# hongfz16/Garment4D

Hardware: AMD Instinct MI355X
Metric: point-cloud frames/s (FPS+ball_query+SA-MLP+LBS), B=8 N=8192 (higher is better)
Workload: dtype f32

## Files before the change

### garment4d_amd/csrc/three_nn_prune.hip

```cpp
#include <cstdlib>

#include "g4d_common.h"
#include "three_nn_body.h"
#include "ball_grid_build.h"

namespace g4d {

namespace {
constexpr int kPrM = 1024;
constexpr int kPrBlk = 16;
constexpr int kPrNB = kPrM / kPrBlk;

__device__ __forceinline__ unsigned pr_part1by2(unsigned v) {
    v &= 0x3ffu;
    v = (v | (v << 16)) & 0x030000ffu;
    v = (v | (v << 8)) & 0x0300f00fu;
    v = (v | (v << 4)) & 0x030c30c3u;
    v = (v | (v << 2)) & 0x09249249u;
    return v;
}

__device__ __forceinline__ float pr_wave_min(float v) {
#pragma unroll
    for (int o = 32; o > 0; o >>= 1) v = fminf(v, __shfl_xor(v, o));
    return v;
}
__device__ __forceinline__ float pr_wave_max(float v) {
#pragma unroll
    for (int o = 32; o > 0; o >>= 1) v = fmaxf(v, __shfl_xor(v, o));
    return v;
}
}

constexpr size_t kPrBoxOff = (size_t)kPrM * 16, kPrCodeOff = kPrBoxOff + (size_t)kPrNB * 32, kPrGridOff = kPrCodeOff + (size_t)kPrNB * 4;
constexpr size_t kPrCloudBytes = kPrGridOff + 16;
constexpr int kPrepT = 512;

__global__ void __launch_bounds__(kPrepT) nn_prune_prep_kernel(int m, const float *__restrict__ known_all, unsigned char *__restrict__ ws) {
    __shared__ unsigned long long keys[kPrM];
    __shared__ float sx[kPrM], sy[kPrM], sz[kPrM];
    __shared__ float red[6][kPrepT / 64];
    const int t = threadIdx.x, lane = t & 63, wave = t >> 6, b = blockIdx.x;
    const float *known = known_all + (size_t)b * m * 3;
    const float INF = __builtin_inff();
    float lx = INF, ly = INF, lz = INF, hx = -INF, hy = -INF, hz = -INF;
    for (int k = t; k < kPrM; k += kPrepT) {
        const bool ok = k < m;
        const float x = ok ? known[k * 3 + 0] : INF, y = ok ? known[k * 3 + 1] : INF, z = ok ? known[k * 3 + 2] : INF;
        sx[k] = x; sy[k] = y; sz[k] = z;
        if (ok && x - x == 0.f && y - y == 0.f && z - z == 0.f) {
            lx = fminf(lx, x); ly = fminf(ly, y); lz = fminf(lz, z);
            hx = fmaxf(hx, x); hy = fmaxf(hy, y); hz = fmaxf(hz, z);
        }
    }
    lx = pr_wave_min(lx); ly = pr_wave_min(ly); lz = pr_wave_min(lz);
    hx = pr_wave_max(hx); hy = pr_wave_max(hy); hz = pr_wave_max(hz);
    if (lane == 0) { red[0][wave] = lx; red[1][wave] = ly; red[2][wave] = lz; red[3][wave] = hx; red[4][wave] = hy; red[5][wave] = hz; }
    __syncthreads();
#pragma unroll
    for (int w = 0; w < kPrepT / 64; ++w) {
        lx = fminf(lx, red[0][w]); ly = fminf(ly, red[1][w]); lz = fminf(lz, red[2][w]);
        hx = fmaxf(hx, red[3][w]); hy = fmaxf(hy, red[4][w]); hz = fmaxf(hz, red[5][w]);
    }
    const float ext = fmaxf(fmaxf(hx - lx, hy - ly), fmaxf(hz - lz, 1e-30f));
    const float scale = ext < INF ? 1023.0f / ext : 0.f;
    for (int k = t; k < kPrM; k += kPrepT) {
        unsigned long long key = ~0ull;
        if (k < m) {
            const float x = sx[k], y = sy[k], z = sz[k];
            const unsigned cx = (unsigned)fminf(fmaxf((x - lx) * scale, 0.f), 1023.f);
            const unsigned cy = (unsigned)fminf(fmaxf((y - ly) * scale, 0.f), 1023.f);
            const unsigned cz = (unsigned)fminf(fmaxf((z - lz) * scale, 0.f), 1023.f);
            const unsigned code = pr_part1by2(cx) | (pr_part1by2(cy) << 1) | (pr_part1by2(cz) << 2);
            key = ((unsigned long long)code << 32) | (unsigned)k;
        }
        keys[k] = key;
    }
    __syncthreads();
    for (int k = 2; k <= kPrM; k <<= 1) {
        for (int j = k >> 1; j > 0; j >>= 1) {
            for (int i = t; i < kPrM / 2; i += kPrepT) {
                const int a = ((i & ~(j - 1)) << 1) | (i & (j - 1));
                const int c = a | j;
                const unsigned long long ka = keys[a], kc = keys[c];
                const bool asc = (a & k) == 0;
                if ((ka > kc) == asc) { keys[a] = kc; keys[c] = ka; }
            }
            __syncthreads();
        }
    }
    float4 *rec = reinterpret_cast<float4 *>(ws + (size_t)b * kPrCloudBytes);
    float *box = reinterpret_cast<float *>(ws + (size_t)b * kPrCloudBytes + kPrBoxOff);
    unsigned *bcode = reinterpret_cast<unsigned *>(ws + (size_t)b * kPrCloudBytes + kPrCodeOff);
    if (t == 0) { float *g = reinterpret_cast<float *>(ws + (size_t)b * kPrCloudBytes + kPrGridOff); g[0] = lx; g[1] = ly; g[2] = lz; g[3] = scale; }
    for (int p = t; p < kPrM; p += kPrepT) {
        const unsigned long long key = keys[p];
        const bool ok = key != ~0ull;
        const int k = ok ? (int)(unsigned)key : 0;
        rec[p] = make_float4(ok ? sx[k] : INF, ok ? sy[k] : INF, ok ? sz[k] : INF, __int_as_float(ok ? k : 0x7fffffff));
    }
    if (t < kPrNB) {
        float bl[3] = {INF, INF, INF}, bh[3] = {-INF, -INF, -INF};
        for (int q = 0; q < kPrBlk; ++q) {
            const unsigned long long key = keys[t * kPrBlk + q];
            if (key == ~0ull) continue;
            const int k = (int)(unsigned)key;
            bl[0] = fminf(bl[0], sx[k]); bl[1] = fminf(bl[1], sy[k]); bl[2] = fminf(bl[2], sz[k]);
            bh[0] = fmaxf(bh[0], sx[k]); bh[1] = fmaxf(bh[1], sy[k]); bh[2] = fmaxf(bh[2], sz[k]);
        }
        bcode[t] = (unsigned)(keys[t * kPrBlk] >> 32);
        float *o = box + t * 8;
        o[0] = bl[0]; o[1] = bl[1]; o[2] = bl[2]; o[3] = 0.f; o[4] = bh[0]; o[5] = bh[1]; o[6] = bh[2]; o[7] = 0.f;
    }
}

__device__ __forceinline__ float pr_gap(float lo, float hi, float qlo, float qhi) { return fmaxf(fmaxf(lo - qhi, qlo - hi), 0.f); }

constexpr int kPrT = 1024;
template <int FM>
__global__ void __launch_bounds__(kPrT) three_nn_prune_kernel(int n, int m, const float *__restrict__ unknown_all, const unsigned char *__restrict__ ws,
                                                            float *__restrict__ dist2_all, int *__restrict__ idx_all,
                                                            const unsigned char *__restrict__ qrec, size_t qstride, int sorted_out) {
    constexpr int LB = kPrBlk + 4;
    __shared__ __attribute__((aligned(16))) float skx[kPrNB * LB], sky[kPrNB * LB], skz[kPrNB * LB];
    __shared__ __attribute__((aligned(16))) int ski[kPrNB * LB];
    __shared__ __attribute__((aligned(16))) float sbox[kPrNB * 8];
    __shared__ unsigned scode[kPrNB];
    __shared__ float sgrid[4];
    const int b = blockIdx.y, t = threadIdx.x, lane = t & 63;
    static_assert(kPrM == kPrT && kPrNB * 8 <= kPrT, "one record per thread");
    const unsigned char *cw = ws + (size_t)b * kPrCloudBytes;
    const float4 r = reinterpret_cast<const float4 *>(cw)[t];
    const float boxv = reinterpret_cast<const float *>(cw + kPrBoxOff)[min(t, kPrNB * 8 - 1)];
    const unsigned codev = reinterpret_cast<const unsigned *>(cw + kPrCodeOff)[min(t, kPrNB - 1)];
    const float gridv = reinterpret_cast<const float *>(cw + kPrGridOff)[min(t, 3)];
    const int p = (int)blockIdx.x * kPrT + t;
    float ux, uy, uz;
    int orig = p;
    if (qrec) {
        const float4 q = reinterpret_cast<const float4 *>(qrec + (size_t)b * qstride)[min(p, n - 1)];
        ux = q.x; uy = q.y; uz = q.z; orig = sorted_out ? p : __float_as_int(q.w);
    } else {
        const float *u = unknown_all + ((size_t)b * n + min(p, n - 1)) * 3;
        ux = u[0]; uy = u[1]; uz = u[2];
    }
    {
        const int jj = (t >> 4) * LB + (t & 15);
        skx[jj] = r.x; sky[jj] = r.y; skz[jj] = r.z; ski[jj] = __float_as_int(r.w);
        if (t < kPrNB * 8) sbox[t] = boxv;
        if (t < kPrNB) scode[t] = codev;
        if (t < 4) sgrid[t] = gridv;
    }
    __syncthreads();
    const float INF = __builtin_inff();
    float b1 = INF, b2 = INF, b3 = INF;
    int i1 = 0, i2 = 0, i3 = 0;
    const int nblk = (m + kPrBlk - 1) / kPrBlk;
    int hb;
    {
        const float gx = sgrid[0], gy = sgrid[1], gz = sgrid[2], gs = sgrid[3];
        const unsigned cx = (unsigned)fminf(fmaxf((ux - gx) * gs, 0.f), 1023.f), cy = (unsigned)fminf(fmaxf((uy - gy) * gs, 0.f), 1023.f),
                       cz = (unsigned)fminf(fmaxf((uz - gz) * gs, 0.f), 1023.f);
        const unsigned cq = pr_part1by2(cx) | (pr_part1by2(cy) << 1) | (pr_part1by2(cz) << 2);
        int pos = 0;
#pragma unroll
        for (int step = kPrNB / 2; step > 0; step >>= 1)
            if (pos + step < nblk && scode[pos + step] <= cq) pos += step;
        hb = pos;
#pragma unroll 4
        for (int s4 = 0; s4 < kPrBlk; ++s4) {
            const int j = hb * LB + s4;
            const float d = dist2<FM>(ux - skx[j], uy - sky[j], uz - skz[j]);
            if (d < INF) nn_insert_lex(d, ski[j], b1, b2, b3, i1, i2, i3);
        }
    }
    const float qlx = pr_wave_min(ux), qly = pr_wave_min(uy), qlz = pr_wave_min(uz);
    const float qhx = pr_wave_max(ux), qhy = pr_wave_max(uy), qhz = pr_wave_max(uz);
    const float *mybox = sbox + min(lane, kPrNB - 1) * 8;
    const float wbound = dist2<FM>(pr_gap(mybox[0], mybox[4], qlx, qhx), pr_gap(mybox[1], mybox[5], qly, qhy), pr_gap(mybox[2], mybox[6], qlz, qhz));
    const bool nanq = !(ux == ux && uy == uy && uz == uz);
    const float maxb3 = pr_wave_max(nanq ? -INF : b3);
    unsigned long long rest = __builtin_amdgcn_ballot_w64(lane < nblk && !(wbound > maxb3));
    for (; rest != 0ull; rest &= rest - 1) {
        const int blk = __builtin_ctzll(rest);
        const float *bx = sbox + blk * 8;
        const float dq = dist2<FM>(pr_gap(bx[0], bx[4], ux, ux), pr_gap(bx[1], bx[5], uy, uy), pr_gap(bx[2], bx[6], uz, uz));
        const bool want = !nanq && blk != hb && !(dq > b3);
        if (__builtin_amdgcn_ballot_w64(want) == 0ull) continue;
#pragma unroll
        for (int s4 = 0; s4 < kPrBlk; s4 += 4) {
            const int j = blk * LB + s4;
            const float4 kx = *reinterpret_cast<const float4 *>(&skx[j]), ky = *reinterpret_cast<const float4 *>(&sky[j]),
                         kz = *reinterpret_cast<const float4 *>(&skz[j]);
            const int4 ki = *reinterpret_cast<const int4 *>(&ski[j]);
            const float d0 = dist2<FM>(ux - kx.x, uy - ky.x, uz - kz.x);
            const float d1 = dist2<FM>(ux - kx.y, uy - ky.y, uz - kz.y);
            const float d2 = dist2<FM>(ux - kx.z, uy - ky.z, uz - kz.z);
            const float d3 = dist2<FM>(ux - kx.w, uy - ky.w, uz - kz.w);
            const bool ok = blk != hb;
            if (__builtin_amdgcn_ballot_w64(ok && fminf(fminf(d0, d1), fminf(d2, d3)) <= b3) == 0ull) continue;
            if (__builtin_amdgcn_ballot_w64(ok && d0 <= b3 && d0 < INF) != 0ull) { if (ok && d0 < INF) nn_insert_lex(d0, ki.x, b1, b2, b3, i1, i2, i3); }
            if (__builtin_amdgcn_ballot_w64(ok && d1 <= b3 && d1 < INF) != 0ull) { if (ok && d1 < INF) nn_insert_lex(d1, ki.y, b1, b2, b3, i1, i2, i3); }
            if (__builtin_amdgcn_ballot_w64(ok && d2 <= b3 && d2 < INF) != 0ull) { if (ok && d2 < INF) nn_insert_lex(d2, ki.z, b1, b2, b3, i1, i2, i3); }
            if (__builtin_amdgcn_ballot_w64(ok && d3 <= b3 && d3 < INF) != 0ull) { if (ok && d3 < INF) nn_insert_lex(d3, ki.w, b1, b2, b3, i1, i2, i3); }
        }
    }
    if (p < n) {
        float *d2o = dist2_all + ((size_t)b * n + orig) * 3;
        int *ix = idx_all + ((size_t)b * n + orig) * 3;
        d2o[0] = b1; d2o[1] = b2; d2o[2] = b3;
        ix[0] = i1; ix[1] = i2; ix[2] = i3;
    }
}

}

using namespace g4d;

extern "C" int g4d_three_nn_pruned_supported(int n, int m) { return n > 0 && m >= 16 && m <= kPrM; }
extern "C" long long g4d_three_nn_pruned_ws_bytes(int b) { return (long long)(b > 0 ? b : 0) * (long long)kPrCloudBytes; }
extern "C" int g4d_three_nn_pruned_f32(int b, int n, int m, const float *unknown, const void *unknown_grid, const float *known, float *dist2, int *idx,
                                       int sorted_out, void *ws, long long ws_bytes, g4d_stream_t stream) {
    G4D_REQUIRE(b >= 0 && b <= 65535 && g4d_three_nn_pruned_supported(n, m), "g4d_three_nn_pruned_f32: needs 16 <= m <= 1024, n > 0, b <= 65535 (use g4d_three_nn_f32)");
    if (b == 0) return G4D_OK;
    G4D_REQUIRE(known && dist2 && idx && ws && (unknown || unknown_grid) && (!sorted_out || unknown_grid), "g4d_three_nn_pruned_f32: null pointer");
    G4D_REQUIRE(ws_bytes >= g4d_three_nn_pruned_ws_bytes(b) && (reinterpret_cast<uintptr_t>(ws) & 15) == 0, "g4d_three_nn_pruned_f32: workspace too small or not 16-byte aligned");
    hipStream_t st = reinterpret_cast<hipStream_t>(stream);
    hipLaunchKernelGGL(nn_prune_prep_kernel, dim3(b), dim3(kPrepT), 0, st, m, known, reinterpret_cast<unsigned char *>(ws));
    if (const int rc = check_launch("g4d_three_nn_pruned_f32(prep)")) return rc;
    size_t off = 0, stride = 0;
    const unsigned char *qrec = nullptr;
    if (unknown_grid) {
        grid_sorted_layout(n, &off, &stride);
        qrec = reinterpret_cast<const unsigned char *>(unknown_grid) + off;
    }
    dim3 grid((n + kPrT - 1) / kPrT, b);
    G4D_WITH_FM(distance_contraction(), hipLaunchKernelGGL((three_nn_prune_kernel<FM>), grid, dim3(kPrT), 0, st, n, m, unknown, reinterpret_cast<const unsigned char *>(ws), dist2, idx,
                                                           qrec, stride, sorted_out))
    return check_launch("g4d_three_nn_pruned_f32");
}
```

Before: 52110.

## Compact per-wave candidate point lists before three-NN refinement in pruned kernel

Replaces the block-by-block refinement loop with a two-round scheme. Each wavefront gathers candidate known points from surviving blocks, filtering them per point against the wave's bounding box and a distance threshold, and writes the survivors into a shared-memory list via ballot/mbcnt compaction. All lanes then scan this dense list. The first round uses the wave-min of the current third-best distance and the second round the wave-max, which aims to reduce wasted distance evaluations and divergence. The cost is extra shared memory (which may lower occupancy), wave-level barriers, and more complex control flow.

```diff
diff --git a/garment4d_amd/csrc/three_nn_prune.hip b/garment4d_amd/csrc/three_nn_prune.hip
--- a/garment4d_amd/csrc/three_nn_prune.hip
+++ b/garment4d_amd/csrc/three_nn_prune.hip
@@ -116,6 +116,13 @@
 
 __device__ __forceinline__ float pr_gap(float lo, float hi, float qlo, float qhi) { return fmaxf(fmaxf(lo - qhi, qlo - hi), 0.f); }
 
+__device__ __forceinline__ void pr_wave_sync() {
+    __builtin_amdgcn_fence(__ATOMIC_RELEASE, "wavefront");
+    __builtin_amdgcn_wave_barrier();
+    __builtin_amdgcn_fence(__ATOMIC_ACQUIRE, "wavefront");
+}
+
+constexpr int kPrList = 128;
 constexpr int kPrT = 1024;
 template <int FM>
 __global__ void __launch_bounds__(kPrT) three_nn_prune_kernel(int n, int m, const float *__restrict__ unknown_all, const unsigned char *__restrict__ ws,
@@ -127,6 +134,8 @@
     __shared__ __attribute__((aligned(16))) float sbox[kPrNB * 8];
     __shared__ unsigned scode[kPrNB];
     __shared__ float sgrid[4];
+    __shared__ __attribute__((aligned(16))) float slx[kPrT / 64 * kPrList], sly[kPrT / 64 * kPrList], slz[kPrT / 64 * kPrList];
+    __shared__ __attribute__((aligned(16))) int sli[kPrT / 64 * kPrList], slb[kPrT / 64 * kPrList];
     const int b = blockIdx.y, t = threadIdx.x, lane = t & 63;
     static_assert(kPrM == kPrT && kPrNB * 8 <= kPrT, "one record per thread");
     const unsigned char *cw = ws + (size_t)b * kPrCloudBytes;
@@ -179,31 +188,60 @@
     const float *mybox = sbox + min(lane, kPrNB - 1) * 8;
     const float wbound = dist2<FM>(pr_gap(mybox[0], mybox[4], qlx, qhx), pr_gap(mybox[1], mybox[5], qly, qhy), pr_gap(mybox[2], mybox[6], qlz, qhz));
     const bool nanq = !(ux == ux && uy == uy && uz == uz);
-    const float maxb3 = pr_wave_max(nanq ? -INF : b3);
-    unsigned long long rest = __builtin_amdgcn_ballot_w64(lane < nblk && !(wbound > maxb3));
-    for (; rest != 0ull; rest &= rest - 1) {
-        const int blk = __builtin_ctzll(rest);
-        const float *bx = sbox + blk * 8;
-        const float dq = dist2<FM>(pr_gap(bx[0], bx[4], ux, ux), pr_gap(bx[1], bx[5], uy, uy), pr_gap(bx[2], bx[6], uz, uz));
-        const bool want = !nanq && blk != hb && !(dq > b3);
-        if (__builtin_amdgcn_ballot_w64(want) == 0ull) continue;
-#pragma unroll
-        for (int s4 = 0; s4 < kPrBlk; s4 += 4) {
-            const int j = blk * LB + s4;
-            const float4 kx = *reinterpret_cast<const float4 *>(&skx[j]), ky = *reinterpret_cast<const float4 *>(&sky[j]),
-                         kz = *reinterpret_cast<const float4 *>(&skz[j]);
-            const int4 ki = *reinterpret_cast<const int4 *>(&ski[j]);
-            const float d0 = dist2<FM>(ux - kx.x, uy - ky.x, uz - kz.x);
-            const float d1 = dist2<FM>(ux - kx.y, uy - ky.y, uz - kz.y);
-            const float d2 = dist2<FM>(ux - kx.z, uy - ky.z, uz - kz.z);
-            const float d3 = dist2<FM>(ux - kx.w, uy - ky.w, uz - kz.w);
-            const bool ok = blk != hb;
-            if (__builtin_amdgcn_ballot_w64(ok && fminf(fminf(d0, d1), fminf(d2, d3)) <= b3) == 0ull) continue;
-            if (__builtin_amdgcn_ballot_w64(ok && d0 <= b3 && d0 < INF) != 0ull) { if (ok && d0 < INF) nn_insert_lex(d0, ki.x, b1, b2, b3, i1, i2, i3); }
-            if (__builtin_amdgcn_ballot_w64(ok && d1 <= b3 && d1 < INF) != 0ull) { if (ok && d1 < INF) nn_insert_lex(d1, ki.y, b1, b2, b3, i1, i2, i3); }
-            if (__builtin_amdgcn_ballot_w64(ok && d2 <= b3 && d2 < INF) != 0ull) { if (ok && d2 < INF) nn_insert_lex(d2, ki.z, b1, b2, b3, i1, i2, i3); }
-            if (__builtin_amdgcn_ballot_w64(ok && d3 <= b3 && d3 < INF) != 0ull) { if (ok && d3 < INF) nn_insert_lex(d3, ki.w, b1, b2, b3, i1, i2, i3); }
-        }
+    const int w = __builtin_amdgcn_readfirstlane(t >> 6), sub = lane >> 4;
+    float *lx = slx + w * kPrList, *ly = sly + w * kPrList, *lz = slz + w * kPrList;
+    int *li = sli + w * kPrList, *lb = slb + w * kPrList;
+    const bool allnan = __builtin_amdgcn_ballot_w64(!nanq) == 0ull;
+    float lo = 0.f;
+#pragma unroll 1
+    for (int round = 0; round < 2 && !allnan; ++round) {
+        const float hi = round == 0 ? pr_wave_min(nanq ? INF : b3) : pr_wave_max(nanq ? -INF : b3);
+        if (round == 1 && !(hi > lo)) break;
+        unsigned long long rest = __builtin_amdgcn_ballot_w64(lane < nblk && !(wbound > hi));
+        int cnt = 0;
+        for (;;) {
+            if (rest == 0ull || cnt > kPrList - 64 - 3) {
+                if (lane < 3) { lx[cnt + lane] = INF; ly[cnt + lane] = INF; lz[cnt + lane] = INF; li[cnt + lane] = 0; lb[cnt + lane] = 0; }
+                pr_wave_sync();
+                for (int j = 0; j < cnt; j += 4) {
+                    const float4 kx = *reinterpret_cast<const float4 *>(&lx[j]), ky = *reinterpret_cast<const float4 *>(&ly[j]),
+                                 kz = *reinterpret_cast<const float4 *>(&lz[j]);
+                    const int4 ki = *reinterpret_cast<const int4 *>(&li[j]), kb = *reinterpret_cast<const int4 *>(&lb[j]);
+                    const float d0 = dist2<FM>(ux - kx.x, uy - ky.x, uz - kz.x);
+                    const float d1 = dist2<FM>(ux - kx.y, uy - ky.y, uz - kz.y);
+                    const float d2 = dist2<FM>(ux - kx.z, uy - ky.z, uz - kz.z);
+                    const float d3 = dist2<FM>(ux - kx.w, uy - ky.w, uz - kz.w);
+                    const float e0 = kb.x != hb ? d0 : INF, e1 = kb.y != hb ? d1 : INF, e2 = kb.z != hb ? d2 : INF, e3 = kb.w != hb ? d3 : INF;
+                    if (__builtin_amdgcn_ballot_w64(fminf(fminf(e0, e1), fminf(e2, e3)) <= b3) == 0ull) continue;
+                    if (__builtin_amdgcn_ballot_w64(e0 <= b3 && e0 < INF) != 0ull) { if (e0 < INF) nn_insert_lex(e0, ki.x, b1, b2, b3, i1, i2, i3); }
+                    if (__builtin_amdgcn_ballot_w64(e1 <= b3 && e1 < INF) != 0ull) { if (e1 < INF) nn_insert_lex(e1, ki.y, b1, b2, b3, i1, i2, i3); }
+                    if (__builtin_amdgcn_ballot_w64(e2 <= b3 && e2 < INF) != 0ull) { if (e2 < INF) nn_insert_lex(e2, ki.z, b1, b2, b3, i1, i2, i3); }
+                    if (__builtin_amdgcn_ballot_w64(e3 <= b3 && e3 < INF) != 0ull) { if (e3 < INF) nn_insert_lex(e3, ki.w, b1, b2, b3, i1, i2, i3); }
+                }
+                pr_wave_sync();
+                cnt = 0;
+                if (rest == 0ull) break;
+            }
+            int blk = -1;
+#pragma unroll
+            for (int g = 0; g < 4; ++g) {
+                const int nb = rest != 0ull ? __builtin_ctzll(rest) : -1;
+                rest &= rest - 1;
+                blk = sub == g ? nb : blk;
+            }
+            const int j = max(blk, 0) * LB + (lane & 15);
+            const float x = skx[j], y = sky[j], z = skz[j];
+            const int ki = ski[j];
+            const float bound = dist2<FM>(pr_gap(x, x, qlx, qhx), pr_gap(y, y, qly, qhy), pr_gap(z, z, qlz, qhz));
+            const bool take = blk >= 0 && ki < m && (round == 0 || bound > lo) && !(bound > hi);
+            const unsigned long long tm = __builtin_amdgcn_ballot_w64(take);
+            if (take) {
+                const int q = cnt + (int)__builtin_amdgcn_mbcnt_hi((unsigned)(tm >> 32), __builtin_amdgcn_mbcnt_lo((unsigned)tm, 0u));
+                lx[q] = x; ly[q] = y; lz[q] = z; li[q] = ki; lb[q] = blk;
+            }
+            cnt += __builtin_popcountll(tm);
+        }
+        lo = hi;
     }
     if (p < n) {
         float *d2o = dist2_all + ((size_t)b * n + orig) * 3;
```

Result: no change. 52310 (median of 4 runs) (+0.4%).
